# Zxhh123/pixel-nerf-multiscale

Measured on AMD Instinct MI355X. Metric: rendered rays/sec (128 samples/ray), SRN chairs 1-view, higher is better.
Workload: dtype fp16; 1 GPU; srn_chairs_1view_128x128_k128; rays_per_gpu=16384, samples_per_ray=128, n_coarse=128, n_fine=0, parallelism=ray-shard x1 + all_gather

## Files before the change

### pixel_nerf_multiscale_amd/csrc/f32_kernels.h

```cpp
#pragma once
#include "pnr_common.h"

namespace pnr {

struct LatCL { const float* p[PNR_MAX_LEVELS]; };
static inline uint64_t latent_cl_bytes(const pnr_views& vw) {
    uint64_t n = 0;
    for (int l = 0; l < vw.n_levels; ++l)
        n += (((uint64_t)vw.n_objs * vw.n_views * vw.lat_c[l] * vw.lat_h[l] * vw.lat_w[l] * 4) + 255) & ~(uint64_t)255;
    return n;
}
static __global__ void k_latent_to_cl(const float* __restrict__ src, int64_t n_views, int C, int T, float* __restrict__ dst) {
    const int64_t e = (int64_t)blockIdx.x * blockDim.x + threadIdx.x;
    if (e >= n_views * C * T) return;
    const int c = (int)(e % C);
    const int64_t r = e / C;
    const int t = (int)(r % T);
    const int64_t v = r / T;
    dst[e] = src[(v * C + c) * T + t];
}
static inline LatCL latent_cl_build(const pnr_views& vw, void* base, hipStream_t s) {
    LatCL cl{};
    uint8_t* p = (uint8_t*)base;
    for (int l = 0; l < vw.n_levels; ++l) {
        if (!vw.latent[l]) return LatCL{};
        const int64_t nv = (int64_t)vw.n_objs * vw.n_views, n = nv * vw.lat_c[l] * vw.lat_h[l] * vw.lat_w[l];
        hipLaunchKernelGGL(k_latent_to_cl, dim3((unsigned)((n + 255) / 256)), dim3(256), 0, s, vw.latent[l], nv, vw.lat_c[l],
                           vw.lat_h[l] * vw.lat_w[l], (float*)p);
        cl.p[l] = (const float*)p;
        p += ((uint64_t)n * 4 + 255) & ~(uint64_t)255;
    }
    return cl;
}

static __global__ void __launch_bounds__(256) k_features_f32(pnr_views vw, PointSrc src, int64_t g0, int CH, int64_t pts_per_obj,
                               int L, int d_in, int use_code_viewdirs, int num_freqs, float freq_factor,
                               float* __restrict__ zx, int ldz , LatCL cl) {
    const int E = L + d_in;
    const int lane = threadIdx.x & 63;
    const int64_t col = (int64_t)blockIdx.x * 4 + (threadIdx.x >> 6);
    if (col >= (int64_t)CH * vw.n_views) return;
    const int v = (int)(col / CH);
    const int pl = (int)(col - (int64_t)v * CH);
    const int64_t g = g0 + pl;
    const int obj = (int)(g / pts_per_obj);
    const int view = obj * vw.n_views + v;
    float p[3], d[3], xr[3], dr[3];
    fetch_point(src, g, p, d);
    const Cam cam = load_cam(vw, view);
    rot3(cam.R, p, xr);
    rot3(cam.R, d, dr);
    float u, w;
    project(cam, xr, u, w);
    float* row = zx + (size_t)col * ldz;
    int e0 = 0;
    for (int lvl = 0; lvl < vw.n_levels; ++lvl) {
        const int W = vw.lat_w[lvl], H = vw.lat_h[lvl], C = vw.lat_c[lvl];
        const Taps t = bilinear_taps(u * uv_sx(vw, lvl), w * uv_sy(vw, lvl), W, H);
        if (cl.p[lvl]) {
            const float* base = cl.p[lvl] + (size_t)view * (size_t)(H * W) * C;
            for (int ch = lane; ch < C; ch += 64) {
                float val = 0.f;
#pragma unroll
                for (int i = 0; i < 4; ++i) val += base[(size_t)t.off[i] * C + ch] * t.w[i];
                row[e0 + ch] = val;
            }
        } else {
            const float* base = vw.latent[lvl] + (size_t)view * C * (size_t)(H * W);
            for (int ch = lane; ch < C; ch += 64) {
                const float* bc = base + (size_t)ch * (size_t)(H * W);
                float val = 0.f;
#pragma unroll
                for (int i = 0; i < 4; ++i) val += bc[t.off[i]] * t.w[i];
                row[e0 + ch] = val;
            }
        }
        e0 += C;
    }
    const float x6[6] = {xr[0], xr[1], xr[2], dr[0], dr[1], dr[2]};
    const int dcode = 3 + 6 * num_freqs;
    for (int j = lane; j < E - L; j += 64) {
        float val;
        if (use_code_viewdirs) val = posenc_elem(x6, 6, j, freq_factor);
        else val = (j < dcode) ? posenc_elem(xr, 3, j, freq_factor) : dr[j - dcode];
        row[L + j] = val;
    }
}

static inline bool latent_width_matches(const pnr_views& vw, int L) {
    int sum = 0;
    for (int i = 0; i < vw.n_levels; ++i) sum += vw.lat_c[i];
    return sum == L;
}
static inline int32_t features_launch(const pnr_views& vw, const PointSrc& src, int64_t g0, int CH, int64_t pts_per_obj, int L, int d_in,
                                      int use_code_viewdirs, int num_freqs, float freq_factor, float* zx, int ldz, hipStream_t s,
                                      LatCL cl = LatCL{}) {
    if (!latent_width_matches(vw, L)) return PNR_E_SHAPE;
    const int64_t cols = (int64_t)CH * vw.n_views;
    if (cols == 0) return PNR_OK;
    hipLaunchKernelGGL(k_features_f32, dim3((unsigned)((cols + 3) / 4)), dim3(256), 0, s, vw, src, g0, CH, pts_per_obj, L, d_in,
                       use_code_viewdirs, num_freqs, freq_factor, zx, ldz, cl);
    return PNR_OK;
}

static __global__ void k_combine_f32(const float* __restrict__ x, int NS, int64_t per_view, int combine_type,
                              float* __restrict__ y) {
    int64_t i = (int64_t)blockIdx.x * blockDim.x + threadIdx.x;
    if (i >= per_view) return;
    float a = x[i];
    if (combine_type == PNR_COMBINE_MAX) {
        for (int v = 1; v < NS; ++v) a = fmaxf(a, x[i + v * per_view]);
    } else {
        for (int v = 1; v < NS; ++v) a += x[i + v * per_view];
        a = a / (float)NS;
    }
    y[i] = a;
}

static __global__ void k_out_act(const float* __restrict__ o, int64_t n, float* __restrict__ out) {
    int64_t i = (int64_t)blockIdx.x * blockDim.x + threadIdx.x;
    if (i >= n) return;
    float4 v = ((const float4*)o)[i];
    v.x = 1.0f / (1.0f + expf(-v.x));
    v.y = 1.0f / (1.0f + expf(-v.y));
    v.z = 1.0f / (1.0f + expf(-v.z));
    v.w = fmaxf(v.w, 0.f);
    ((float4*)out)[i] = v;
}

}
```

### pixel_nerf_multiscale_amd/csrc/point_f32.hip

```cpp
#include "f32_kernels.h"

namespace pnr {

int32_t linear_f32_mfma(const float* X, int ldx, const float* W, int ldw, const float* b, bool relu_in, bool accum, float* Y,
                        int ldy, int64_t M, int N, int K, hipStream_t s);

template <bool RELU_IN, bool ACCUM>
static int32_t linear(const float* X, int ldx, const float* W, const float* b, float* Y, int ldy, int M, int N, int K,
                      hipStream_t s) {
    return linear_f32_mfma(X, ldx, W, K, b, RELU_IN, ACCUM, Y, ldy, M, N, K, s);
}

static const int F32_CHUNK = 49152;

uint64_t point_f32_workspace_bytes(const pnr_mlp* mlp, const pnr_views* vw) {
    uint64_t per_pt = (uint64_t)vw->n_views * (feature_stride(mlp) + 2ull * mlp->d_hidden) + 4;
    return per_pt * F32_CHUNK * sizeof(float) + 512 + latent_cl_bytes(*vw);
}

static int32_t chain_f32(const pnr_mlp* mlp, const float* zx, int E, int CH, int NS, float* x, float* h, float* o, hipStream_t s) {
    const int L = mlp->d_latent, Din = mlp->d_in, H = mlp->d_hidden;
    const int nz = n_lin_z(mlp);
    int M = CH * NS;
    int32_t rc;
    if ((rc = linear<false, false>(zx + L, E, mlp->lin_in_w, mlp->lin_in_b, x, H, M, H, Din, s))) return rc;
    for (int b = 0; b < mlp->n_blocks; ++b) {
        if (b == mlp->combine_layer && NS > 1) {
            int64_t per_view = (int64_t)CH * H;
            hipLaunchKernelGGL(k_combine_f32, dim3((unsigned)((per_view + 255) / 256)), dim3(256), 0, s, x, NS,
                               per_view, mlp->combine_type, x);
            PNR_LAUNCH_CHECK();
            M = CH;
        }
        if (L > 0 && b < nz)
            if ((rc = linear<false, true>(zx, E, mlp->lin_z_w[b], mlp->lin_z_b[b], x, H, M, H, L, s))) return rc;
        if ((rc = linear<true, false>(x, H, mlp->fc0_w[b], mlp->fc0_b[b], h, H, M, H, H, s))) return rc;
        if ((rc = linear<true, true>(h, H, mlp->fc1_w[b], mlp->fc1_b[b], x, H, M, H, H, s))) return rc;
    }
    if (M != CH) return PNR_E_UNSUPPORTED;
    return linear<true, false>(x, H, mlp->lin_out_w, mlp->lin_out_b, o, mlp->d_out, M, mlp->d_out, H, s);
}

int32_t point_f32(const pnr_params* prm, const pnr_mlp* mlp, const pnr_views* vw, PointSrc src, int64_t n_points,
                  int64_t pts_per_obj, float* out, void* workspace, uint64_t ws_bytes, hipStream_t s) {
    if (ws_bytes < point_f32_workspace_bytes(mlp, vw)) return PNR_E_WORKSPACE;
    if (mlp->d_out != 4) return PNR_E_SHAPE;
    const int NS = vw->n_views, L = mlp->d_latent, Din = mlp->d_in, H = mlp->d_hidden;
    const int E = feature_stride(mlp);
    float* zx = (float*)round_up_256(workspace);
    float* x = zx + (size_t)F32_CHUNK * NS * E;
    float* h = x + (size_t)F32_CHUNK * NS * H;
    float* o4 = h + (size_t)F32_CHUNK * NS * H;
    void* cl_base = round_up_256(o4 + (size_t)F32_CHUNK * 4);
    const LatCL cl = (L > 0 && n_points >= 4096) ? latent_cl_build(*vw, cl_base, s) : LatCL{};
    PNR_LAUNCH_CHECK();
    for (int64_t g0 = 0; g0 < n_points; g0 += F32_CHUNK) {
        int CH = (int)((n_points - g0 < F32_CHUNK) ? (n_points - g0) : F32_CHUNK);
        PNR_TRY(features_launch(*vw, src, g0, CH, pts_per_obj, L, Din, prm->use_code_viewdirs, prm->num_freqs, prm->freq_factor, zx, E, s, cl));
        PNR_LAUNCH_CHECK();
        int32_t rc;
        if ((rc = chain_f32(mlp, zx, E, CH, NS, x, h, o4, s))) return rc;
        hipLaunchKernelGGL(k_out_act, dim3((unsigned)((CH + 255) / 256)), dim3(256), 0, s, o4, (int64_t)CH, out + g0 * 4);
        PNR_LAUNCH_CHECK();
    }
    return PNR_OK;
}

uint64_t resnetfc_f32_workspace_bytes(const pnr_mlp* mlp, int NS) {
    uint64_t per_pt = (uint64_t)NS * (mlp->d_latent + mlp->d_in + 2ull * mlp->d_hidden);
    return per_pt * F32_CHUNK * sizeof(float) + 256;
}
int32_t resnetfc_f32(const pnr_mlp* mlp, const float* zx, int64_t outer, int NS, int64_t B, float* out, void* workspace,
                     uint64_t ws_bytes, hipStream_t s) {
    if (ws_bytes < resnetfc_f32_workspace_bytes(mlp, NS)) return PNR_E_WORKSPACE;
    const int H = mlp->d_hidden, E = mlp->d_latent + mlp->d_in;
    float* zc = (float*)round_up_256(workspace);
    float* x = zc + (size_t)F32_CHUNK * NS * E;
    float* h = x + (size_t)F32_CHUNK * NS * H;
    for (int64_t o = 0; o < outer; ++o)
        for (int64_t p0 = 0; p0 < B; p0 += F32_CHUNK) {
            const int CH = (int)((B - p0 < F32_CHUNK) ? (B - p0) : F32_CHUNK);
            const float* src = zx + ((size_t)o * NS * B + p0) * E;
            const float* rows = src;
            if (NS > 1 && CH != B) {
                PNR_HIP_CHECK(hipMemcpy2DAsync(zc, (size_t)CH * E * 4, src, (size_t)B * E * 4, (size_t)CH * E * 4, NS,
                                               hipMemcpyDeviceToDevice, s));
                rows = zc;
            }
            int32_t rc;
            if ((rc = chain_f32(mlp, rows, E, CH, NS, x, h, out + ((size_t)o * B + p0) * mlp->d_out, s))) return rc;
        }
    return PNR_OK;
}

static __global__ void k_index_latent(pnr_views vw, const float* __restrict__ uv, int64_t N, int uv_views, int L,
                                      float* __restrict__ out) {
    const int64_t idx = (int64_t)blockIdx.x * blockDim.x + threadIdx.x;
    const int64_t V = (int64_t)vw.n_objs * vw.n_views;
    if (idx >= V * L * N) return;
    const int64_t n = idx % N;
    const int e = (int)((idx / N) % L);
    const int64_t view = idx / (N * L);
    const float* q = uv + ((uv_views == 1 ? 0 : view) * N + n) * 2;
    int lvl = 0, ch = e;
    while (ch >= vw.lat_c[lvl]) { ch -= vw.lat_c[lvl]; ++lvl; }
    const int W = vw.lat_w[lvl], H = vw.lat_h[lvl], C = vw.lat_c[lvl];
    const Taps t = bilinear_taps(q[0] * uv_sx(vw, lvl), q[1] * uv_sy(vw, lvl), W, H);
    const float* base = vw.latent[lvl] + ((size_t)view * C + ch) * (size_t)(H * W);
    float val = 0.f;
#pragma unroll
    for (int i = 0; i < 4; ++i) val += base[t.off[i]] * t.w[i];
    out[idx] = val;
}
int32_t index_latent_f32(const pnr_views* vw, const float* uv, int64_t N, int uv_views, float* out, hipStream_t s) {
    int L = 0;
    for (int i = 0; i < vw->n_levels; ++i) L += vw->lat_c[i];
    const int64_t tot = (int64_t)vw->n_objs * vw->n_views * L * N;
    if (tot == 0) return PNR_OK;
    hipLaunchKernelGGL(k_index_latent, dim3((unsigned)((tot + 255) / 256)), dim3(256), 0, s, *vw, uv, N, uv_views, L, out);
    PNR_LAUNCH_CHECK();
    return PNR_OK;
}

}
```

Baseline: 1.977 million rays/s.

## Precompute lin_z projections per texel and bilinearly sample projected maps

Because bilinear sampling is linear, the per-block latent projection (lin_z) is now applied once to every texel of each latent level, producing H-wide projected maps. Per point, the feature kernel then writes only the projected uv plus the positional encoding, and a new kernel bilinearly samples the projected maps and adds them to the hidden state. This removes the per-point M×H×L GEMM for each lin_z block and the wide latent row, in exchange for extra workspace, an upfront GEMM over all texels, and gathers that are H wide instead of C wide. It is gated on large point counts where the number of points exceeds the number of texels.

Measured after the change: 1.975 million rays/s, median of 2. No clear change (-0.1%).

```diff
diff --git a/pixel_nerf_multiscale_amd/csrc/f32_kernels.h b/pixel_nerf_multiscale_amd/csrc/f32_kernels.h
--- a/pixel_nerf_multiscale_amd/csrc/f32_kernels.h
+++ b/pixel_nerf_multiscale_amd/csrc/f32_kernels.h
@@ -35,7 +35,7 @@
 
 static __global__ void __launch_bounds__(256) k_features_f32(pnr_views vw, PointSrc src, int64_t g0, int CH, int64_t pts_per_obj,
                                int L, int d_in, int use_code_viewdirs, int num_freqs, float freq_factor,
-                               float* __restrict__ zx, int ldz , LatCL cl) {
+                               float* __restrict__ zx, int ldz , LatCL cl, int uv_rows) {
     const int E = L + d_in;
     const int lane = threadIdx.x & 63;
     const int64_t col = (int64_t)blockIdx.x * 4 + (threadIdx.x >> 6);
@@ -54,7 +54,8 @@
     project(cam, xr, u, w);
     float* row = zx + (size_t)col * ldz;
     int e0 = 0;
-    for (int lvl = 0; lvl < vw.n_levels; ++lvl) {
+    if (uv_rows && lane == 0) { row[0] = u; row[1] = w; }
+    for (int lvl = 0; lvl < (uv_rows ? 0 : vw.n_levels); ++lvl) {
         const int W = vw.lat_w[lvl], H = vw.lat_h[lvl], C = vw.lat_c[lvl];
         const Taps t = bilinear_taps(u * uv_sx(vw, lvl), w * uv_sy(vw, lvl), W, H);
         if (cl.p[lvl]) {
@@ -79,12 +80,62 @@
     }
     const float x6[6] = {xr[0], xr[1], xr[2], dr[0], dr[1], dr[2]};
     const int dcode = 3 + 6 * num_freqs;
+    const int c0 = uv_rows ? 2 : L;
     for (int j = lane; j < E - L; j += 64) {
         float val;
         if (use_code_viewdirs) val = posenc_elem(x6, 6, j, freq_factor);
         else val = (j < dcode) ? posenc_elem(xr, 3, j, freq_factor) : dr[j - dcode];
-        row[L + j] = val;
+        row[c0 + j] = val;
     }
+}
+
+struct LinZMaps { const float* base; uint64_t per_block; uint64_t off[PNR_MAX_LEVELS]; };
+static inline uint64_t lin_z_maps_floats_per_block(const pnr_views& vw, int H) {
+    uint64_t texels = 0;
+    for (int l = 0; l < vw.n_levels; ++l) texels += (uint64_t)vw.lat_h[l] * vw.lat_w[l];
+    return (uint64_t)vw.n_objs * vw.n_views * texels * H;
+}
+
+template <int VEC>
+static __global__ void __launch_bounds__(256) k_add_lin_z_f32(pnr_views vw, int64_t g0, int CH, int64_t pts_per_obj,
+                               const float* __restrict__ zx, int ldz, const float* __restrict__ P ,
+                               LinZMaps maps, const float* __restrict__ bias, int H, float* __restrict__ x) {
+    const int lane = threadIdx.x & 63;
+    const int64_t col = (int64_t)blockIdx.x * 4 + (threadIdx.x >> 6);
+    if (col >= (int64_t)CH * vw.n_views) return;
+    const int v = (int)(col / CH);
+    const int pl = (int)(col - (int64_t)v * CH);
+    const int obj = (int)((g0 + pl) / pts_per_obj);
+    const int view = obj * vw.n_views + v;
+    const float u = zx[(size_t)col * ldz], w = zx[(size_t)col * ldz + 1];
+    float* xr = x + (size_t)col * H;
+    typedef float fv __attribute__((ext_vector_type(VEC)));
+    for (int h = lane * VEC; h < H; h += 64 * VEC) {
+        fv acc = *(const fv*)(bias + h);
+        for (int lvl = 0; lvl < vw.n_levels; ++lvl) {
+            const int Wl = vw.lat_w[lvl], Hl = vw.lat_h[lvl];
+            const Taps t = bilinear_taps(u * uv_sx(vw, lvl), w * uv_sy(vw, lvl), Wl, Hl);
+            const float* base = P + maps.off[lvl] + (size_t)view * (size_t)(Hl * Wl) * H + h;
+#pragma unroll
+            for (int i = 0; i < 4; ++i) {
+                const fv p = *(const fv*)(base + (size_t)t.off[i] * H);
+                acc = __builtin_elementwise_fma((fv)t.w[i], p, acc);
+            }
+        }
+        *(fv*)(xr + h) = *(const fv*)(xr + h) + acc;
+    }
+}
+static inline int32_t add_lin_z_launch(const pnr_views& vw, int64_t g0, int CH, int64_t pts_per_obj, const float* zx, int ldz,
+                                       const LinZMaps& maps, int b, const float* bias, int H, float* x, hipStream_t s) {
+    const int64_t cols = (int64_t)CH * vw.n_views;
+    if (cols == 0) return PNR_OK;
+    const float* P = maps.base + (size_t)b * maps.per_block;
+    const dim3 grid((unsigned)((cols + 3) / 4)), blk(256);
+    if (H % 4 == 0 && (((uintptr_t)bias | (uintptr_t)P | (uintptr_t)x) & 15) == 0)
+        hipLaunchKernelGGL((k_add_lin_z_f32<4>), grid, blk, 0, s, vw, g0, CH, pts_per_obj, zx, ldz, P, maps, bias, H, x);
+    else
+        hipLaunchKernelGGL((k_add_lin_z_f32<1>), grid, blk, 0, s, vw, g0, CH, pts_per_obj, zx, ldz, P, maps, bias, H, x);
+    return PNR_OK;
 }
 
 static inline bool latent_width_matches(const pnr_views& vw, int L) {
@@ -94,12 +145,12 @@
 }
 static inline int32_t features_launch(const pnr_views& vw, const PointSrc& src, int64_t g0, int CH, int64_t pts_per_obj, int L, int d_in,
                                       int use_code_viewdirs, int num_freqs, float freq_factor, float* zx, int ldz, hipStream_t s,
-                                      LatCL cl = LatCL{}) {
+                                      LatCL cl = LatCL{}, bool uv_rows = false) {
     if (!latent_width_matches(vw, L)) return PNR_E_SHAPE;
     const int64_t cols = (int64_t)CH * vw.n_views;
     if (cols == 0) return PNR_OK;
     hipLaunchKernelGGL(k_features_f32, dim3((unsigned)((cols + 3) / 4)), dim3(256), 0, s, vw, src, g0, CH, pts_per_obj, L, d_in,
-                       use_code_viewdirs, num_freqs, freq_factor, zx, ldz, cl);
+                       use_code_viewdirs, num_freqs, freq_factor, zx, ldz, cl, uv_rows ? 1 : 0);
     return PNR_OK;
 }
 
diff --git a/pixel_nerf_multiscale_amd/csrc/point_f32.hip b/pixel_nerf_multiscale_amd/csrc/point_f32.hip
--- a/pixel_nerf_multiscale_amd/csrc/point_f32.hip
+++ b/pixel_nerf_multiscale_amd/csrc/point_f32.hip
@@ -13,17 +13,48 @@
 
 static const int F32_CHUNK = 49152;
 
+static uint64_t lin_z_maps_bytes(const pnr_mlp* mlp, const pnr_views* vw) {
+    if (mlp->d_latent <= 0) return 0;
+    return round_up_256((uint64_t)n_lin_z(mlp) * lin_z_maps_floats_per_block(*vw, mlp->d_hidden) * sizeof(float));
+}
+
 uint64_t point_f32_workspace_bytes(const pnr_mlp* mlp, const pnr_views* vw) {
     uint64_t per_pt = (uint64_t)vw->n_views * (feature_stride(mlp) + 2ull * mlp->d_hidden) + 4;
-    return per_pt * F32_CHUNK * sizeof(float) + 512 + latent_cl_bytes(*vw);
+    return per_pt * F32_CHUNK * sizeof(float) + 768 + latent_cl_bytes(*vw) +
+           lin_z_maps_bytes(mlp, vw);
 }
 
-static int32_t chain_f32(const pnr_mlp* mlp, const float* zx, int E, int CH, int NS, float* x, float* h, float* o, hipStream_t s) {
+static int32_t lin_z_maps_build(const pnr_mlp* mlp, const pnr_views& vw, const LatCL& cl, float* base, LinZMaps* maps, hipStream_t s) {
+    const int H = mlp->d_hidden, L = mlp->d_latent;
+    const int64_t nv = (int64_t)vw.n_objs * vw.n_views;
+    uint64_t off = 0;
+    for (int l = 0; l < vw.n_levels; ++l) {
+        maps->off[l] = off;
+        off += (uint64_t)nv * vw.lat_h[l] * vw.lat_w[l] * H;
+    }
+    maps->base = base;
+    maps->per_block = off;
+    for (int b = 0; b < n_lin_z(mlp); ++b) {
+        int ch0 = 0;
+        for (int l = 0; l < vw.n_levels; ++l) {
+            const int C = vw.lat_c[l];
+            PNR_TRY(linear_f32_mfma(cl.p[l], C, mlp->lin_z_w[b] + ch0, L, nullptr, false, false, base + (size_t)b * off + maps->off[l], H,
+                                    nv * vw.lat_h[l] * vw.lat_w[l], H, C, s));
+            ch0 += C;
+        }
+    }
+    return PNR_OK;
+}
+
+struct LinZApply { const pnr_views* vw; int64_t g0, pts_per_obj; const LinZMaps* maps; };
+
+static int32_t chain_f32(const pnr_mlp* mlp, const float* zx, int E, int CH, int NS, float* x, float* h, float* o, hipStream_t s,
+                         const LinZApply* pz = nullptr) {
     const int L = mlp->d_latent, Din = mlp->d_in, H = mlp->d_hidden;
     const int nz = n_lin_z(mlp);
     int M = CH * NS;
     int32_t rc;
-    if ((rc = linear<false, false>(zx + L, E, mlp->lin_in_w, mlp->lin_in_b, x, H, M, H, Din, s))) return rc;
+    if ((rc = linear<false, false>(zx + (pz ? 2 : L), E, mlp->lin_in_w, mlp->lin_in_b, x, H, M, H, Din, s))) return rc;
     for (int b = 0; b < mlp->n_blocks; ++b) {
         if (b == mlp->combine_layer && NS > 1) {
             int64_t per_view = (int64_t)CH * H;
@@ -32,8 +63,12 @@
             PNR_LAUNCH_CHECK();
             M = CH;
         }
-        if (L > 0 && b < nz)
-            if ((rc = linear<false, true>(zx, E, mlp->lin_z_w[b], mlp->lin_z_b[b], x, H, M, H, L, s))) return rc;
+        if (L > 0 && b < nz) {
+            if (pz) {
+                if ((rc = add_lin_z_launch(*pz->vw, pz->g0, CH, pz->pts_per_obj, zx, E, *pz->maps, b, mlp->lin_z_b[b], H, x, s))) return rc;
+                PNR_LAUNCH_CHECK();
+            } else if ((rc = linear<false, true>(zx, E, mlp->lin_z_w[b], mlp->lin_z_b[b], x, H, M, H, L, s))) return rc;
+        }
         if ((rc = linear<true, false>(x, H, mlp->fc0_w[b], mlp->fc0_b[b], h, H, M, H, H, s))) return rc;
         if ((rc = linear<true, true>(h, H, mlp->fc1_w[b], mlp->fc1_b[b], x, H, M, H, H, s))) return rc;
     }
@@ -54,12 +89,20 @@
     void* cl_base = round_up_256(o4 + (size_t)F32_CHUNK * 4);
     const LatCL cl = (L > 0 && n_points >= 4096) ? latent_cl_build(*vw, cl_base, s) : LatCL{};
     PNR_LAUNCH_CHECK();
+    int64_t texels = 0;
+    for (int l = 0; l < vw->n_levels; ++l) texels += (int64_t)vw->lat_h[l] * vw->lat_w[l];
+    const bool projected = L > 0 && cl.p[0] && n_lin_z(mlp) > 0 && n_points >= F32_CHUNK && n_points >= texels;
+    LinZMaps maps{};
+    if (projected) PNR_TRY(lin_z_maps_build(mlp, *vw, cl, (float*)round_up_256((uint8_t*)cl_base + latent_cl_bytes(*vw)), &maps, s));
+    const int Ez = projected ? ((Din + 2 + 3) & ~3) : E;
     for (int64_t g0 = 0; g0 < n_points; g0 += F32_CHUNK) {
         int CH = (int)((n_points - g0 < F32_CHUNK) ? (n_points - g0) : F32_CHUNK);
-        PNR_TRY(features_launch(*vw, src, g0, CH, pts_per_obj, L, Din, prm->use_code_viewdirs, prm->num_freqs, prm->freq_factor, zx, E, s, cl));
+        PNR_TRY(features_launch(*vw, src, g0, CH, pts_per_obj, L, Din, prm->use_code_viewdirs, prm->num_freqs, prm->freq_factor, zx, Ez, s, cl,
+                                projected));
         PNR_LAUNCH_CHECK();
         int32_t rc;
-        if ((rc = chain_f32(mlp, zx, E, CH, NS, x, h, o4, s))) return rc;
+        const LinZApply pz{vw, g0, pts_per_obj, &maps};
+        if ((rc = chain_f32(mlp, zx, Ez, CH, NS, x, h, o4, s, projected ? &pz : nullptr))) return rc;
         hipLaunchKernelGGL(k_out_act, dim3((unsigned)((CH + 255) / 256)), dim3(256), 0, s, o4, (int64_t)CH, out + g0 * 4);
         PNR_LAUNCH_CHECK();
     }
```
